# shubhamchandak94/Spring

Hardware: AMD Instinct MI355X
Metric: Mreads/s through reorder stage (higher is better)
Workload: dtype u64; 1 GPU; 100000000 x 150 bp single-end synthetic reads per GPU (uniform genome 600000000 bp, 25x coverage, 1.0% substitutions, 50% reverse-complemented), inputs resident in HBM as .dna records; reads_per_gpu=100000000, read_len=150, chains=65536, num_thr=8, parallelism=single GPU, unmatched=13958636, singletons=12720853, rounds=1984, chain_groups=2

## Files before the change

### include/spring_reorder.h

```cpp
#ifndef SPRING_REORDER_H_
#define SPRING_REORDER_H_

#include <stddef.h>
#include <stdint.h>

#ifdef __cplusplus
extern "C" {
#endif

#define SPRING_REORDER_E_ARG (-1)
#define SPRING_REORDER_E_IO (-2)
#define SPRING_REORDER_E_HIP (-3)
#define SPRING_REORDER_E_STATE (-4)

typedef struct spring_reorder_ctx spring_reorder_ctx;

typedef struct {
  int32_t device;
  uint32_t num_chains;
  int32_t num_thr;
  int32_t collect_stats;
  int32_t time_search;
  int32_t force_literal_update;
  int32_t rounds_per_sync;
// ... 10 lines not shown
  int32_t devices[8];
  int32_t mg_host_transport;
  int32_t table_mode;
  int32_t plan0[6];
  int32_t plan1[6];
  int32_t long_min;
  int32_t long_blocks;
  int32_t debug;
  int32_t long_split;
  int32_t entry_flags;
  int32_t out_writers;
  int32_t alternatives;
  int32_t phases;
  int32_t known_absent;
  int32_t sort_prefix_bits;
} spring_reorder_opts;

typedef struct {
  uint64_t n_reads, n_matched, n_single, unmatched;
  uint64_t probes, keyok, cands, hits, iterations, rounds, lost;
  uint64_t numkeys[2], dict_numreads[2];
  double ms_unpack, ms_dict, ms_chains, ms_finalize, ms_total;
  double ms_search_kernel;
  uint64_t search_launches;
  uint64_t device_bytes;
  double ms_exchange, ms_resolve_mark;
  uint64_t chains;
  uint64_t deep_pool;
  uint64_t long_searches;
  uint64_t table_minz;
  uint64_t table_marked_lines;
  uint64_t long_splits;
  uint64_t alternatives;
  uint64_t phases;
  double ms_search_busy;
  uint64_t sort_prefix_bits;
  uint64_t sort_repaired_runs;
  uint64_t sort_full_sorts;
  uint64_t sort_long_runs;
  uint64_t sort_list_overflows;
} spring_reorder_stats;

void spring_reorder_default_opts(spring_reorder_opts *o);
const char *spring_reorder_last_error(void);
void spring_reorder_trim_pool(void);

int spring_reorder_run(const char *temp_dir, uint32_t max_readlen, int32_t num_thr, int32_t paired_end,
                       uint32_t num_reads_clean_0, uint32_t num_reads_clean_1,
                       const spring_reorder_opts *opts );

int spring_reorder_create(spring_reorder_ctx **ctx, const spring_reorder_opts *opts);
void spring_reorder_destroy(spring_reorder_ctx *ctx);

int spring_reorder_load_dna(spring_reorder_ctx *ctx, const uint8_t *dna, size_t nbytes, uint32_t n,
                            uint32_t max_readlen);
// ... 82 lines not shown
```

### spring_amd/_lib.py

```python
import ctypes as C
import os

HERE = os.path.dirname(os.path.abspath(__file__))
LIB_PATH = os.environ.get("SPRING_AMD_LIB") or os.path.join(HERE, "lib", "libspring_reorder_hip.so")

EXPORTS = [
    "spring_reorder_default_opts", "spring_reorder_last_error", "spring_reorder_trim_pool", "spring_reorder_run", "spring_reorder_create",
    "spring_reorder_destroy", "spring_reorder_load_dna", "spring_reorder_load_dna_device",
    "spring_reorder_build_dict", "spring_reorder_run_chains", "spring_reorder_auto_chains", "spring_reorder_finalize",
    "spring_reorder_mg_begin", "spring_reorder_mg_search", "spring_reorder_mg_slice", "spring_reorder_mg_slices",
    "spring_reorder_mg_apply",
    "spring_reorder_mg_end", "spring_reorder_mg_exchange_virtual", "spring_reorder_debug_check_seed_state",
    "spring_mg_rccl_unique_id", "spring_mg_comm_create_rccl", "spring_mg_comm_create_host", "spring_mg_comm_destroy",
    "spring_reorder_mg_run",
    "spring_reorder_get_stats", "spring_reorder_download", "spring_reorder_tid_split", "spring_reorder_emit_dna",
    "spring_reorder_dict_lookup", "spring_reorder_download_reads", "spring_synth_dna_bytes",
    "spring_reorder_load_fastq", "spring_reorder_fastq_N",
    "spring_order_invert_se", "spring_order_invert_pe", "spring_order_correct", "spring_order_pe_encode",
    "spring_fastq_reorder",
    "spring_synth_dna_host", "spring_synth_genome_host", "spring_synth_dna_device", "spring_reorder_load_synth", "spring_reorder_download_dna",
    "spring_encoder_create", "spring_encoder_destroy", "spring_encoder_set_split_tables", "spring_encoder_encode_reorder", "spring_encoder_download",
    "spring_encoder_download_seq_packed", "spring_encoder_get_info", "spring_reorder_encode_run", "spring_encoder_encode_host", "spring_encoder_run",
]

# ... 20 lines not shown
    "spring_fastq_out_write", "spring_fastq_out_get_info",
]


class Opts(C.Structure):
    _fields_ = [("device", C.c_int32), ("num_chains", C.c_uint32), ("num_thr", C.c_int32),
                ("collect_stats", C.c_int32), ("time_search", C.c_int32), ("force_literal_update", C.c_int32),
                ("rounds_per_sync", C.c_int32), ("long_budget", C.c_int32),
                ("first_shifts", C.c_int32), ("seed_wide", C.c_int32), ("tab_scale", C.c_int32),
                ("search_wpb", C.c_int32), ("dbg_search_lds", C.c_int32), ("dbg_apply_lds", C.c_int32),
                ("fused", C.c_int32), ("deep_bins", C.c_int32),
                ("num_devices", C.c_int32), ("devices", C.c_int32 * 8), ("mg_host_transport", C.c_int32),
                ("table_mode", C.c_int32), ("plan0", C.c_int32 * 6), ("plan1", C.c_int32 * 6), ("long_min", C.c_int32),
                ("long_blocks", C.c_int32), ("debug", C.c_int32), ("long_split", C.c_int32), ("entry_flags", C.c_int32),
                ("out_writers", C.c_int32), ("alternatives", C.c_int32), ("phases", C.c_int32), ("known_absent", C.c_int32),
                ("sort_prefix_bits", C.c_int32)]


class FastqInfo(C.Structure):
    _fields_ = [("num_reads", C.c_uint32 * 2), ("num_reads_clean", C.c_uint32 * 2), ("num_reads_N", C.c_uint32 * 2),
                ("max_readlen", C.c_uint32), ("pad", C.c_uint32), ("ms_device", C.c_double)]


class EncoderInfo(C.Structure):
    _fields_ = ([(k, C.c_uint64) for k in ("n_aligned", "n_total", "seq_len", "noise_bytes", "n_noisepos",
                                           "unaligned_bytes", "len_unaligned", "num_contigs")]
                + [(k, C.c_uint32) for k in ("matched_s", "matched_N", "align_passes", "max_bin")]
                + [("ms_device", C.c_double), ("ms_phase", C.c_double * 8)])

    def asdict(self):
        d = {}
# ... 63 lines not shown
        return d


class Stats(C.Structure):
    _fields_ = ([(k, C.c_uint64) for k in ("n_reads", "n_matched", "n_single", "unmatched", "probes", "keyok",
                                          "cands", "hits", "iterations", "rounds", "lost")]
                + [("numkeys", C.c_uint64 * 2), ("dict_numreads", C.c_uint64 * 2)]
                + [(k, C.c_double) for k in ("ms_unpack", "ms_dict", "ms_chains", "ms_finalize", "ms_total",
                                             "ms_search_kernel")]
                + [("search_launches", C.c_uint64), ("device_bytes", C.c_uint64),
                   ("ms_exchange", C.c_double), ("ms_resolve_mark", C.c_double), ("chains", C.c_uint64),
                   ("deep_pool", C.c_uint64), ("long_searches", C.c_uint64),
                   ("table_minz", C.c_uint64), ("table_marked_lines", C.c_uint64), ("long_splits", C.c_uint64), ("alternatives", C.c_uint64), ("phases", C.c_uint64),
                   ("ms_search_busy", C.c_double),
                   ("sort_prefix_bits", C.c_uint64), ("sort_repaired_runs", C.c_uint64), ("sort_full_sorts", C.c_uint64),
                   ("sort_long_runs", C.c_uint64), ("sort_list_overflows", C.c_uint64)])

    def asdict(self):
        d = {}
        for k, _ in self._fields_:
            v = getattr(self, k)
            d[k] = list(v) if hasattr(v, "__len__") else v
        return d


MG_ALLGATHER_FN = C.CFUNCTYPE(C.c_int, C.c_void_p, C.c_size_t, C.c_size_t, C.c_size_t, C.c_void_p)

_lib = None


def lib():
# ... 137 lines not shown
```

### spring_amd/build.py

```python
import os
import subprocess
import sys

HERE = os.path.dirname(os.path.abspath(__file__))
ROOT = os.path.dirname(HERE)
CSRC = os.path.join(HERE, "csrc")
LIBDIR = os.path.join(HERE, "lib")
LIB = os.path.join(LIBDIR, "libspring_reorder_hip.so")
SOURCES = ["reorder_kernels.hip", "reorder_pipeline.cpp", "reorder_files.cpp", "order_ops.hip", "fastq_kernels.hip",
           "encoder.hip", "fastq_reorder.hip", "streams.hip", "decode.hip", "qualid.hip", "fastq_out.hip"]
HEADERS = ["reorder_device.h", "reorder_internal.h", "reorder_round_mc.h", "synth_common.h", "call_reorder.h",
           "encoder_internal.h", "streams_internal.h", "fastq_out_internal.h"]
PUBLIC_HEADERS = ["spring_reorder.h", "spring_encoder.h", "spring_streams.h", "spring_decode.h", "spring_qualid.h",
                  "spring_fastq_out.h"]


def _stale():
    if not os.path.exists(LIB):
        return True
    t = os.path.getmtime(LIB)
    deps = [os.path.join(CSRC, f) for f in SOURCES + HEADERS] + [os.path.join(ROOT, "include", h) for h in PUBLIC_HEADERS]
    return any(os.path.getmtime(d) > t for d in deps)


def build(force=False, verbose=False):
    if not force and not _stale():
        return LIB
# ... 28 lines not shown
```

### spring_amd/csrc/reorder_pipeline.cpp

```cpp
#include <hip/hip_runtime.h>
#include <dlfcn.h>

#include <algorithm>
#include <system_error>
#include <thread>
#include <memory>
#include <atomic>
#include <chrono>
#include <cstdarg>
#include <cstdio>
#include <cstdlib>
#include <cstring>
#include <map>
#include <mutex>
#include <new>
#include <stdexcept>
#include <string>
#include <unordered_map>
#include <vector>
#include <zlib.h>

#include "reorder_device.h"
#include "reorder_internal.h"
#include "spring_reorder.h"
#include "synth_common.h"

namespace sr {
thread_local std::string g_err;
int fail(int code, const char *fmt, ...) {
  char buf[512];
  va_list ap;
  va_start(ap, fmt);
  vsnprintf(buf, sizeof(buf), fmt, ap);
  va_end(ap);
  g_err = buf;
  return code;
}
// ... 73 lines not shown
  spring_reorder_opts o;
  int dev = 0;
  hipStream_t st = nullptr;
  int stage = ST_CREATED;
  std::vector<void *> allocs;
  uint64_t dev_bytes = 0, peak_bytes = 0;
  uint8_t *d_dna = nullptr;
  bool dna_borrowed = false;
  size_t dna_bytes = 0;
  uint64_t *d_off = nullptr;
  uint32_t n = 0;
  int L = 0, W = 0, S = 0, Lpad = 0;
  bool uniform = true;
  uint64_t *d_reads = nullptr;
  uint16_t *d_lens = nullptr;
  DictDev dict[2];
  uint4 *fpt = nullptr;
  int bshift = 63;
  int minz = 0, lshift = 31;
  uint32_t marked_lines = 0;
  bool user_plan0 = false;
  DevParams P;
  uint32_t K = 0;
  uint64_t nrec = 0, nsing = 0, cap = 0;
  bool mg = false;
  uint32_t *cnt_buf[2] = {nullptr, nullptr};
  uint64_t round_no = 0;
  hipStream_t st2 = nullptr, st3 = nullptr;
  uint64_t *taken2 = nullptr;
  uint32_t *resv2 = nullptr, *won = nullptr;
// ... 187 lines not shown
    if (p.free_blocks.empty()) continue;
    (void)hipSetDevice(d);
    for (auto &kv : p.free_blocks) { (void)hipFree(kv.second); p.sizes.erase(kv.second); }
    p.free_blocks.clear();
    p.cached = 0;
  }
}

int spring_reorder_create(spring_reorder_ctx **out, const spring_reorder_opts *opts) {
  if (!out) return fail(SPRING_REORDER_E_ARG, "ctx is NULL");
  spring_reorder_opts o;
  if (opts) o = *opts; else spring_reorder_default_opts(&o);
  if (o.num_thr <= 0) return fail(SPRING_REORDER_E_ARG, "num_thr must be >= 1");
  if (o.sort_prefix_bits < 0 || o.sort_prefix_bits > 64)
    return fail(SPRING_REORDER_E_ARG, "sort_prefix_bits: 0 (library's choice) or 1 .. 64 bits of the key hash (64 = the full sort)");
  int ndev = 0;
  HIPCHK(hipGetDeviceCount(&ndev));
  if (ndev <= 0) return fail(SPRING_REORDER_E_HIP, "no HIP device");
  int dev = o.device;
  if (dev < 0) HIPCHK(hipGetDevice(&dev));
  if (dev >= ndev) return fail(SPRING_REORDER_E_ARG, "device %d out of range (%d devices)", dev, ndev);
  HIPCHK(hipSetDevice(dev));
  spring_reorder_ctx *ctx = new spring_reorder_ctx();
  ctx->o = o;
  ctx->dev = dev;
  memset(&ctx->P, 0, sizeof(ctx->P));
  memset(&ctx->stats, 0, sizeof(ctx->stats));
  HIPCHK(hipStreamCreateWithFlags(&ctx->st, hipStreamNonBlocking));
  for (auto &e : ctx->ev) HIPCHK(hipEventCreate(&e));
  ctx->ev_ok = true;
// ... 21 lines not shown
  ctx->n = n;
  ctx->L = (int)max_readlen;
  ctx->W = (2 * ctx->L - 1) / 64 + 1;
  int S = 1;
  while (S < ctx->W) S <<= 1;
  ctx->S = S;
  ctx->Lpad = (ctx->L + 63) / 64 * 64;
  const int L = ctx->L;
  ctx->dict[0].start = L > 100 ? L / 2 - 32 : L / 2 - L * 32 / 100;
  ctx->dict[0].end = L / 2 - 1;
  ctx->dict[1].start = L / 2;
  ctx->dict[1].end = L > 100 ? L / 2 - 1 + 32 : L / 2 - 1 + L * 32 / 100;
  return 0;
}

static int unpack_on_device(spring_reorder_ctx *ctx, uint32_t *d_bad_len = nullptr) {
  if (!ctx->d_reads) DMALLOC(ctx->d_reads, (size_t)std::max<uint32_t>(ctx->n, 1) * ctx->S * sizeof(uint64_t));
  if (!ctx->d_lens) DMALLOC(ctx->d_lens, (size_t)std::max<uint32_t>(ctx->n, 1) * sizeof(uint16_t));
  HIPCHK(hipEventRecord(ctx->ev[0], ctx->st));
  const uint32_t rec = 2u + ((uint32_t)ctx->L + 3u) / 4u;
  launch_unpack(ctx->st, ctx->d_dna, ctx->d_off, ctx->n, ctx->L, ctx->W, ctx->S, rec, ctx->d_reads, ctx->d_lens, d_bad_len);
  HIPCHK(hipGetLastError());
  HIPCHK(hipEventRecord(ctx->ev[1], ctx->st));
  ctx->stage = ST_LOADED;
  return 0;
}

static int upload_chunked(spring_reorder_ctx *ctx, uint8_t *d_dst, size_t nbytes,
                          int (*fill)(void *, size_t, void *, size_t), void *self) {
  if (!nbytes) return 0;
  const size_t nchunks = (nbytes + PIN_CHUNK - 1) / PIN_CHUNK;
  const unsigned hw = std::max(1u, std::thread::hardware_concurrency());
  const int nthr = (int)std::min<size_t>(std::min<size_t>(8, hw), nchunks);
  std::atomic<size_t> next{0};
  std::atomic<int> rc{0};
  std::vector<std::string> errs((size_t)nthr);
// ... 98 lines not shown
int load_dna_source(spring_reorder_ctx *ctx, const DnaSource &src, uint32_t n, uint32_t max_readlen) {
  if (!ctx || !src.fill) return fail(SPRING_REORDER_E_ARG, "NULL argument");
  if (ctx->stage != ST_CREATED) return fail(SPRING_REORDER_E_STATE, "load_dna: context already loaded");
  HIPCHK(hipSetDevice(ctx->dev));
  int r = setup_geometry(ctx, n, max_readlen);
  if (r) return r;
  const size_t rec = 2u + (max_readlen + 3u) / 4u, nbytes = src.nbytes;
  if (n && nbytes == (size_t)n * rec) {
    ctx->uniform = true;
    ctx->dna_bytes = nbytes;
    DMALLOC(ctx->d_dna, nbytes + 16);
    if ((r = upload_chunked(ctx, ctx->d_dna, nbytes, src.fill, src.self))) return r;
    uint32_t *d_bad = nullptr, bad = 0;
    DMALLOC(d_bad, 16);
    HIPCHK(hipMemsetAsync(d_bad, 0, 4, ctx->st));
    if ((r = unpack_on_device(ctx, d_bad))) return r;
    HIPCHK(hipMemcpyAsync(&bad, d_bad, 4, hipMemcpyDeviceToHost, ctx->st));
    HIPCHK(hipStreamSynchronize(ctx->st));
    ctx->dfree(d_bad);
    if (!bad) return 0;
    ctx->stage = ST_CREATED;
    ctx->dfree(ctx->d_dna); ctx->d_dna = nullptr;
  }
  if (src.image) {
    ctx->in_source_fallback = true;
    r = spring_reorder_load_dna(ctx, src.image, nbytes, n, max_readlen);
    ctx->in_source_fallback = false;
    return r;
  }
  std::unique_ptr<uint8_t[]> img;
  try { img.reset(new uint8_t[nbytes + 1]); } catch (const std::bad_alloc &) { return fail(SPRING_REORDER_E_IO, "out of host memory for a %zu-byte record stream", nbytes); }
  {
    const size_t CH = (size_t)64 << 20, nch = (nbytes + CH - 1) / CH;
    const int nthr = (int)std::min<size_t>(std::min<size_t>(8, std::max(1u, std::thread::hardware_concurrency())), std::max<size_t>(nch, 1));
    std::atomic<size_t> next{0};
    std::atomic<int> rc{0};
// ... 56 lines not shown
    return rs;
  }
  int r = setup_geometry(ctx, n, max_readlen);
  if (r) return r;
  std::vector<uint64_t> off;
  r = scan_records(dna, nbytes, n, ctx->L, ctx->uniform, off);
  if (r) return r;
  ctx->dna_bytes = nbytes;
  DMALLOC(ctx->d_dna, nbytes + 16);
  auto mem_fill = [](void *self, size_t o, void *dst, size_t len) -> int { memcpy(dst, (const uint8_t *)self + o, len); return 0; };
  if ((r = upload_chunked(ctx, ctx->d_dna, nbytes, mem_fill, const_cast<uint8_t *>(dna)))) return r;
  if (!ctx->uniform) {
    DMALLOC(ctx->d_off, (size_t)n * sizeof(uint64_t));
    if ((r = upload_chunked(ctx, (uint8_t *)ctx->d_off, (size_t)n * sizeof(uint64_t), mem_fill, off.data()))) return r;
  }
  return unpack_on_device(ctx);
}

int spring_reorder_load_dna_device(spring_reorder_ctx *ctx, const void *d_dna, size_t nbytes, uint32_t n,
                                   uint32_t max_readlen, int32_t fixed_len) {
  if (!ctx) return fail(SPRING_REORDER_E_ARG, "ctx is NULL");
  if (ctx->stage != ST_CREATED) return fail(SPRING_REORDER_E_STATE, "load_dna_device: context already loaded");
  HIPCHK(hipSetDevice(ctx->dev));
  int r = setup_geometry(ctx, n, max_readlen);
  if (r) return r;
  if (fixed_len) {
    const size_t rec = 2u + (max_readlen + 3u) / 4u;
    if (nbytes < rec * n) return fail(SPRING_REORDER_E_ARG, "device stream too short for %u fixed records", n);
    ctx->uniform = true;
    ctx->d_dna = (uint8_t *)d_dna;
    ctx->dna_borrowed = true;
    ctx->dna_bytes = nbytes;
    return unpack_on_device(ctx);
  }
  std::vector<uint8_t> h(nbytes);
  if (nbytes) HIPCHK(hipMemcpy(h.data(), d_dna, nbytes, hipMemcpyDeviceToHost));
  return spring_reorder_load_dna(ctx, h.data(), nbytes, n, max_readlen);
}

namespace {
struct FqFile {
  uint8_t *d_txt = nullptr;
  uint64_t nbytes = 0, nlines = 0, nreads = 0;
  uint64_t *line_end = nullptr;
  uint32_t *len = nullptr, *fclean = nullptr, *szc = nullptr, *fN = nullptr, *szN = nullptr, *cidx = nullptr, *nidx = nullptr;
  uint64_t *coff = nullptr, *noff = nullptr;
  uint32_t n_clean = 0, n_N = 0, maxlen = 0, min_clean = 0xffffffffu;
  uint64_t clean_bytes = 0, N_bytes = 0;
// ... 274 lines not shown

int spring_reorder_load_synth(spring_reorder_ctx *ctx, uint32_t n, uint32_t L, uint64_t G, uint64_t seed,
                              uint32_t err_ppm) {
  if (!ctx) return fail(SPRING_REORDER_E_ARG, "ctx is NULL");
  if (ctx->stage != ST_CREATED) return fail(SPRING_REORDER_E_STATE, "load_synth: context already loaded");
  if (L == 0 || L > (uint32_t)MAX_READ_LEN || G < L) return fail(SPRING_REORDER_E_ARG, "bad synth geometry");
  if ((err_ppm & SYN_PAIRED_FLAG) && (n & 1)) return fail(SPRING_REORDER_E_ARG, "a paired pool holds an even number of reads");
  HIPCHK(hipSetDevice(ctx->dev));
  int r = setup_geometry(ctx, n, L);
  if (r) return r;
  ctx->uniform = true;
  ctx->dna_bytes = spring_synth_dna_bytes(n, L);
  DMALLOC(ctx->d_dna, ctx->dna_bytes + 16);
  launch_synth(ctx->st, ctx->d_dna, n, L, G, seed, syn_err_thr24(err_ppm));
  HIPCHK(hipGetLastError());
  return unpack_on_device(ctx);
}

int spring_reorder_download_dna(spring_reorder_ctx *ctx, uint8_t *dst, size_t cap) {
  if (!ctx || ctx->stage < ST_LOADED) return fail(SPRING_REORDER_E_STATE, "download_dna: nothing loaded");
  if (cap < ctx->dna_bytes) return fail(SPRING_REORDER_E_ARG, "buffer too small");
  HIPCHK(hipSetDevice(ctx->dev));
  HIPCHK(hipStreamSynchronize(ctx->st));
  if (ctx->dna_bytes) HIPCHK(hipMemcpy(dst, ctx->d_dna, ctx->dna_bytes, hipMemcpyDeviceToHost));
  return 0;
}

int spring_reorder_download_reads(spring_reorder_ctx *ctx, uint64_t *limbs, uint16_t *len) {
  if (!ctx || ctx->stage < ST_LOADED) return fail(SPRING_REORDER_E_STATE, "download_reads: nothing loaded");
  HIPCHK(hipSetDevice(ctx->dev));
  HIPCHK(hipStreamSynchronize(ctx->st));
// ... 30 lines not shown

int spring_reorder_build_dict(spring_reorder_ctx *ctx) {
  double t_last = now_ms();
  if (!ctx) return fail(SPRING_REORDER_E_ARG, "ctx is NULL");
  const bool dbg = ctx->o.debug != 0;
  if (ctx->stage != ST_LOADED) return fail(SPRING_REORDER_E_STATE, "build_dict: load reads first");
  HIPCHK(hipSetDevice(ctx->dev));
  hipStream_t st = ctx->st;
  const uint32_t n = ctx->n;
  HIPCHK(hipEventRecord(ctx->ev[2], st));
  uint64_t *uhash[2] = {nullptr, nullptr};
  uint32_t *ustart[2] = {nullptr, nullptr}, *ucount[2] = {nullptr, nullptr};
  const bool both_dense = n && ctx->uniform && ctx->L > ctx->dict[0].end && ctx->L > ctx->dict[1].end;
  uint64_t *keys_both[2] = {nullptr, nullptr};
  uint32_t *vals_both[2] = {nullptr, nullptr};
  ctx->stats.sort_repaired_runs = 0; ctx->stats.sort_full_sorts = 0; ctx->stats.sort_prefix_bits = 0;
  ctx->stats.sort_long_runs = 0; ctx->stats.sort_list_overflows = 0;
  for (int l = 0; l < 2; l++) {
    DictDev &d = ctx->dict[l];
    uint32_t m = 0;
    uint32_t *d_slot = nullptr, *d_flag = nullptr;
    void *d_tmp = nullptr;
    size_t tmp_bytes = 0;
    if (n) {
      if (ctx->uniform) {
        m = ctx->L > d.end ? n : 0;
      } else {
        DMALLOC(d_flag, (size_t)n * 4);
        DMALLOC(d_slot, (size_t)n * 4);
        launch_flag_in_dict(st, ctx->d_lens, n, d.end, d_flag);
// ... 17 lines not shown
      DMALLOC(d.deep, 16);
      DMALLOC(d.d_ndeep, 16);
      HIPCHK(hipMemsetAsync(d.d_ndeep, 0, 12, st));
      if (d_flag) { ctx->dfree(d_flag); ctx->dfree(d_slot); }
      continue;
    }
    uint64_t *k_in = keys_both[l], *k_out = nullptr;
    uint32_t *v_in = vals_both[l], *cnt = nullptr, *d_nruns = nullptr;
    if (!k_in) {
      DMALLOC(k_in, (size_t)m * 8);
      DMALLOC(v_in, (size_t)m * 4);
    }
    DMALLOC(k_out, (size_t)m * 8);
    DMALLOC(d.ids, (size_t)m * 4);
    DBG_T("alloc keys");
    if (l == 0 && both_dense) {
      DMALLOC(keys_both[1], (size_t)n * 8);
      DMALLOC(vals_both[1], (size_t)n * 4);
      launch_keys2(st, ctx->d_reads, n, ctx->S, d.start, d.end, ctx->dict[1].start, ctx->dict[1].end, k_in, v_in,
                   keys_both[1], vals_both[1]);
    } else if (!keys_both[l]) {
      launch_keys(st, ctx->d_reads, ctx->d_lens, ctx->uniform ? nullptr : d_slot, n, ctx->S, d.start, d.end, k_in, v_in);
    }
    HIPCHK(hipGetLastError());
    DBG_T("k_keys");
    const unsigned T = ctx->o.sort_prefix_bits > 0 ? (unsigned)ctx->o.sort_prefix_bits : sort_prefix_auto(m);
    ctx->stats.sort_prefix_bits = T;
    bool full = T >= 64;
    if (!full) {
      uint32_t *d_ctr = nullptr, *d_list = nullptr;
      uint2 *d_runs = nullptr;
// ... 59 lines not shown
    HIPCHK(hipMemsetAsync(d.d_ndeep, 0, 12, st));
    HIPCHK(hipStreamSynchronize(st));
    ctx->dfree(d_tmp);
    if (d_flag) { ctx->dfree(d_flag); ctx->dfree(d_slot); }
  }
  const uint64_t nk0 = ctx->dict[0].numkeys, nk1 = ctx->dict[1].numkeys, nm = nk0 + nk1;
  const int tab_scale = ctx->o.tab_scale > 0 ? ctx->o.tab_scale : 2;
  const uint64_t nb = std::max<uint64_t>(8, pow2ceil(std::max<uint64_t>(2, (nm * 10 + 15) / 16)) * (uint64_t)pow2ceil(tab_scale));
  ctx->bshift = 64;
  for (uint64_t v = nb; v > 1; v >>= 1) ctx->bshift--;
  ctx->minz = (ctx->dict[0].end - ctx->dict[0].start + 1 == MINZ_WL && ctx->L <= 192 && ctx->o.table_mode == 2) ? 1 : 0;
  ctx->lshift = 32 - (64 - ctx->bshift - 2);
  if (ctx->lshift < 1) return fail(SPRING_REORDER_E_ARG, "build_dict: table too large for minimizer addressing");
  ctx->stats.table_minz = ctx->minz; ctx->stats.table_marked_lines = 0;
  DMALLOC(ctx->fpt, nb * 32);
  HIPCHK(hipMemsetAsync(ctx->fpt, 0, nb * 32, st));
  uint32_t *const tab_words = reinterpret_cast<uint32_t *>(ctx->fpt);
  DBG_T("alloc+memset tab");
  if (nm) {
    uint64_t *mv0 = nullptr, *mh = nullptr, *mv = nullptr;
    void *d_tmp = nullptr;
    const uint64_t *h_in = nullptr, *v_in = nullptr;
    if (nk0 && nk1) {
      DMALLOC(mh, nm * 8);
      DMALLOC(mv, nm * 8);
      size_t tb = 0;
      HIPCHK(merge_by_hash(st, nullptr, tb, uhash[0], uhash[1], 1ull << 63, mh, mv, nk0, nk1));
      DMALLOC(d_tmp, tb);
      HIPCHK(merge_by_hash(st, d_tmp, tb, uhash[0], uhash[1], 1ull << 63, mh, mv, nk0, nk1));
      h_in = mh; v_in = mv;
    } else {
      DMALLOC(mv0, nm * 8);
      launch_iota_tag(st, mv0, nm, nk0 ? 0ull : 1ull << 63);
      h_in = nk0 ? uhash[0] : uhash[1];
// ... 1410 lines not shown
```

### spring_amd/reorder.py

```python
import ctypes as C
from dataclasses import dataclass

import numpy as np

from . import _lib


class ReorderError(RuntimeError):
    """Raised where the reference throws std::runtime_error (call_template_functions.cpp:60)."""


@dataclass
class ReorderOpts:
    device: int = -1
    num_chains: int = 0
    num_thr: int = 1
    collect_stats: bool = False
    time_search: bool = False
    force_literal_update: bool = False
    rounds_per_sync: int = 0
    first_shifts: int = 0
    seed_wide: int = 0
    tab_scale: int = 0
    search_wpb: int = 0
# ... 5 lines not shown
    devices: tuple = ()
    mg_host_transport: bool = False
    plan0: tuple = ()
    plan1: tuple = ()
    long_min: int = 0
    long_blocks: int = 0
    entry_flags: int = 0
    long_split: int = 0
    debug: bool = False
    out_writers: int = 0
    alternatives: int = 0
    table_mode: int = 0
    phases: int = 0
    known_absent: int = 0
    sort_prefix_bits: int = 0

    def to_c(self):
        o = _lib.Opts()
        _lib.lib().spring_reorder_default_opts(C.byref(o))
        o.device, o.num_chains, o.num_thr = self.device, self.num_chains, self.num_thr
        o.collect_stats, o.time_search = int(self.collect_stats), int(self.time_search)
        o.force_literal_update, o.rounds_per_sync = int(self.force_literal_update), self.rounds_per_sync
        o.first_shifts, o.seed_wide, o.tab_scale = self.first_shifts, self.seed_wide, self.tab_scale
        o.search_wpb, o.dbg_search_lds, o.dbg_apply_lds = self.search_wpb, self.dbg_search_lds, self.dbg_apply_lds
        o.fused, o.deep_bins = self.fused, self.deep_bins
        o.long_budget = self.long_budget
        if len(self.devices) > 8:
            raise ValueError("at most 8 devices")
        o.table_mode = self.table_mode
        for i, v in enumerate(tuple(self.plan0)[:6]):
            o.plan0[i] = int(v)
        for i, v in enumerate(tuple(self.plan1)[:6]):
            o.plan1[i] = int(v)
        o.long_min, o.long_blocks, o.debug = self.long_min, self.long_blocks, int(self.debug)
        o.long_split, o.entry_flags = self.long_split, self.entry_flags
        o.out_writers = self.out_writers
        o.alternatives = self.alternatives
        o.phases = self.phases
        o.known_absent = self.known_absent
        o.sort_prefix_bits = self.sort_prefix_bits
        o.num_devices = len(self.devices)
        for i, d in enumerate(self.devices):
            o.devices[i] = d
        o.mg_host_transport = int(self.mg_host_transport)
        return o


def _chk(rc):
    if rc != 0:
        raise ReorderError("%s (code %d)" % (_lib.lib().spring_reorder_last_error().decode(), rc))


class ReorderStage:

    def __init__(self, opts: ReorderOpts = None):
# ... 179 lines not shown
```

Measured before the change: 336.8 Mreads/s.

## Fuse dict key generation into unpack and build hash table in one pass

Unpacking fixed-length reads now also emits mixed dictionary keys and ids for both dictionaries in the same kernel, so the separate key-extraction pass over the unpacked reads is skipped. The fingerprint table is built by range-partitioned workgroups that assemble their bucket image in LDS and write it out whole. This replaces the memset plus merge-sort and scatter path, and buckets that run past four slots go to an overflow insert with linear probing. The cost is extra device memory held for the precomputed keys between load and build, plus a new fallback path for overflow entries.

```diff
diff --git a/include/spring_reorder.h b/include/spring_reorder.h
--- a/include/spring_reorder.h
+++ b/include/spring_reorder.h
@@ -48,6 +48,7 @@
   int32_t phases;
   int32_t known_absent;
   int32_t sort_prefix_bits;
+  int32_t dict_build_mode;
 } spring_reorder_opts;
 
 typedef struct {
@@ -73,6 +74,7 @@
   uint64_t sort_full_sorts;
   uint64_t sort_long_runs;
   uint64_t sort_list_overflows;
+  uint64_t dict_build_path;
 } spring_reorder_stats;
 
 void spring_reorder_default_opts(spring_reorder_opts *o);
diff --git a/spring_amd/_lib.py b/spring_amd/_lib.py
--- a/spring_amd/_lib.py
+++ b/spring_amd/_lib.py
@@ -58,7 +58,7 @@
                 ("table_mode", C.c_int32), ("plan0", C.c_int32 * 6), ("plan1", C.c_int32 * 6), ("long_min", C.c_int32),
                 ("long_blocks", C.c_int32), ("debug", C.c_int32), ("long_split", C.c_int32), ("entry_flags", C.c_int32),
                 ("out_writers", C.c_int32), ("alternatives", C.c_int32), ("phases", C.c_int32), ("known_absent", C.c_int32),
-                ("sort_prefix_bits", C.c_int32)]
+                ("sort_prefix_bits", C.c_int32), ("dict_build_mode", C.c_int32)]
 
 
 class FastqInfo(C.Structure):
@@ -152,7 +152,7 @@
                    ("table_minz", C.c_uint64), ("table_marked_lines", C.c_uint64), ("long_splits", C.c_uint64), ("alternatives", C.c_uint64), ("phases", C.c_uint64),
                    ("ms_search_busy", C.c_double),
                    ("sort_prefix_bits", C.c_uint64), ("sort_repaired_runs", C.c_uint64), ("sort_full_sorts", C.c_uint64),
-                   ("sort_long_runs", C.c_uint64), ("sort_list_overflows", C.c_uint64)])
+                   ("sort_long_runs", C.c_uint64), ("sort_list_overflows", C.c_uint64), ("dict_build_path", C.c_uint64)])
 
     def asdict(self):
         d = {}
diff --git a/spring_amd/build.py b/spring_amd/build.py
--- a/spring_amd/build.py
+++ b/spring_amd/build.py
@@ -8,9 +8,9 @@
 LIBDIR = os.path.join(HERE, "lib")
 LIB = os.path.join(LIBDIR, "libspring_reorder_hip.so")
 SOURCES = ["reorder_kernels.hip", "reorder_pipeline.cpp", "reorder_files.cpp", "order_ops.hip", "fastq_kernels.hip",
-           "encoder.hip", "fastq_reorder.hip", "streams.hip", "decode.hip", "qualid.hip", "fastq_out.hip"]
+           "encoder.hip", "fastq_reorder.hip", "streams.hip", "decode.hip", "qualid.hip", "fastq_out.hip", "dict_build.hip"]
 HEADERS = ["reorder_device.h", "reorder_internal.h", "reorder_round_mc.h", "synth_common.h", "call_reorder.h",
-           "encoder_internal.h", "streams_internal.h", "fastq_out_internal.h"]
+           "encoder_internal.h", "streams_internal.h", "fastq_out_internal.h", "dict_build.h"]
 PUBLIC_HEADERS = ["spring_reorder.h", "spring_encoder.h", "spring_streams.h", "spring_decode.h", "spring_qualid.h",
                   "spring_fastq_out.h"]
 
diff --git a/spring_amd/csrc/dict_build.h b/spring_amd/csrc/dict_build.h
--- /dev/null
+++ b/spring_amd/csrc/dict_build.h
@@ -0,0 +1,28 @@
+#ifndef SPRING_DICT_BUILD_H_
+#define SPRING_DICT_BUILD_H_
+
+#include "reorder_device.h"
+
+namespace sr {
+
+bool launch_unpack_keys(hipStream_t st, const uint8_t *dna, uint32_t n, int L, int W, int S, uint32_t rec_fixed,
+                        uint64_t *reads, uint16_t *lens, uint32_t *bad_len, int dstart0, int dend0, int dstart1, int dend1,
+                        uint64_t *keys0, uint32_t *vals0, uint64_t *keys1, uint32_t *vals1);
+
+constexpr int TAB_WRITE_LG = 10;
+inline int tab_write_lg(int bshift) { return 64 - bshift < TAB_WRITE_LG ? 64 - bshift : TAB_WRITE_LG; }
+inline uint32_t tab_write_blocks(int bshift) { return (uint32_t)(1ull << (64 - bshift - tab_write_lg(bshift))); }
+void launch_tab_partition(hipStream_t st, const uint64_t *h0, uint32_t nk0, const uint64_t *h1, uint32_t nk1, int bshift,
+                          uint32_t *part);
+constexpr uint32_t TAB_OVF_SLOTS = 8;
+void launch_tab_write(hipStream_t st, const uint64_t *h0, uint32_t nk0, const uint64_t *h1, uint32_t nk1,
+                      const uint32_t *part, DictBuild d0, DictBuild d1, uint4 *fpt, int bshift, uint32_t *ovf,
+                      uint32_t *ovf_blk, uint32_t *ovf_cnt);
+void launch_tab_overflow_blocks(hipStream_t st, const uint64_t *h0, uint32_t nk0, const uint64_t *h1, DictBuild d0,
+                                DictBuild d1, uint32_t *fpt, int bshift, const uint32_t *ovf_blk, const uint32_t *ovf_cnt);
+void launch_tab_overflow_pairs(hipStream_t st, const uint64_t *h0, uint32_t nk0, const uint64_t *h1, DictBuild d0,
+                               DictBuild d1, uint32_t *fpt, int bshift, const uint32_t *ovf, uint32_t novf);
+
+}
+
+#endif
diff --git a/spring_amd/csrc/dict_build.hip b/spring_amd/csrc/dict_build.hip
--- /dev/null
+++ b/spring_amd/csrc/dict_build.hip
@@ -0,0 +1,289 @@
+#include <hip/hip_runtime.h>
+
+#include "dict_build.h"
+
+namespace sr {
+
+__device__ __forceinline__ uint64_t db_mix64(uint64_t x) {
+  x ^= x >> 33; x *= 0xff51afd7ed558ccdull; x ^= x >> 33; x *= 0xc4ceb9fe1a85ec53ull; x ^= x >> 33;
+  return x;
+}
+__device__ __forceinline__ uint64_t db_unmix64(uint64_t x) {
+  x ^= x >> 33; x *= 0x9cb4b2f8129337dbull; x ^= x >> 33; x *= 0x4f74430c22a54005ull; x ^= x >> 33;
+  return x;
+}
+__device__ __forceinline__ uint32_t db_fp30_of(uint64_t h) {
+  const uint32_t f = (uint32_t)h & 0x3fffffffu;
+  return f == 0u ? 1u : f == 0x3fffffffu ? 0x3ffffffeu : f;
+}
+
+__global__ __launch_bounds__(256) void k_unpack_fixed_keys(const uint8_t *__restrict__ dna, uint32_t n, int L, int W, int lgS,
+                                                           uint32_t rec, uint64_t *__restrict__ reads,
+                                                           uint16_t *__restrict__ lens, uint32_t *__restrict__ bad_len,
+                                                           int dstart0, int klen0, int dstart1, int klen1,
+                                                           uint64_t *__restrict__ keys0, uint32_t *__restrict__ vals0,
+                                                           uint64_t *__restrict__ keys1, uint32_t *__restrict__ vals1) {
+  extern __shared__ uint4 s_unpack[];
+  const uint32_t r0 = blockIdx.x * (uint32_t)UNPACK_READS;
+  const uint32_t nr = min((uint32_t)UNPACK_READS, n - r0);
+  const uint8_t *g = dna + (uint64_t)r0 * rec;
+  const uint32_t sh = (uint32_t)((uintptr_t)g & 15u);
+  const uint4 *ga = reinterpret_cast<const uint4 *>(g - sh);
+  const uint32_t nchunk = (sh + nr * rec + 15u) >> 4;
+  for (uint32_t k = threadIdx.x; k < nchunk; k += 256) s_unpack[k] = ga[k];
+  __syncthreads();
+  const uint8_t *sb = reinterpret_cast<const uint8_t *>(s_unpack);
+  const uint32_t *sw = reinterpret_cast<const uint32_t *>(s_unpack);
+  const bool chk = bad_len != nullptr;
+  const uint32_t S = 1u << lgS;
+  auto len_of = [&](uint32_t r) -> uint32_t {
+    const uint32_t p = sh + r * rec;
+    return (uint32_t)sb[p] | ((uint32_t)sb[p + 1] << 8);
+  };
+  auto limb = [&](uint32_t m) -> uint64_t {
+    const uint32_t r = m >> lgS, j = m & (S - 1u);
+    if ((int)j >= W) return 0;
+    uint32_t len = len_of(r);
+    if (chk && len != (uint32_t)L) len = (uint32_t)L;
+    const uint32_t nb = min((len + 3u) / 4u, rec - 2u), pos = 8u * j;
+    if (pos >= nb) return 0;
+    const uint32_t p = sh + r * rec + 2u + pos, k = p >> 2, s8 = (p & 3u) * 8u;
+    uint64_t v = (uint64_t)sw[k] | ((uint64_t)sw[k + 1] << 32);
+    if (s8) v = (v >> s8) | ((uint64_t)sw[k + 2] << (64u - s8));
+    if (nb - pos < 8u) v &= (1ull << (8u * (nb - pos))) - 1ull;
+    return v;
+  };
+  for (uint32_t t = threadIdx.x; 2u * t < nr; t += 256) {
+    const uint32_t r = 2u * t;
+    uint32_t l0 = len_of(r), l1 = r + 1 < nr ? len_of(r + 1) : (uint32_t)L;
+    if (chk && (l0 != (uint32_t)L || l1 != (uint32_t)L)) {
+      *bad_len = 1u;
+      l0 = l1 = (uint32_t)L;
+    }
+    if (r + 1 < nr) *reinterpret_cast<uint32_t *>(lens + r0 + r) = l0 | (l1 << 16);
+    else lens[r0 + r] = (uint16_t)l0;
+  }
+  const uint32_t nl = nr << lgS;
+  uint64_t *out = reads + ((uint64_t)r0 << lgS);
+  for (uint32_t q = threadIdx.x; 2u * q < nl; q += 256) {
+    const uint32_t m = 2u * q;
+    const uint64_t v0 = limb(m);
+    if (m + 1 < nl) *reinterpret_cast<ulonglong2 *>(out + m) = make_ulonglong2(v0, limb(m + 1));
+    else out[m] = v0;
+  }
+  auto window = [&](uint32_t r, int dstart, int klen2) -> uint64_t {
+    const uint32_t bitpos = 2u * (uint32_t)dstart, li = bitpos >> 6, off = bitpos & 63u;
+    uint64_t v = limb((r << lgS) + li) >> off;
+    if (off && li + 1u < S) v |= limb((r << lgS) + li + 1u) << (64u - off);
+    if (klen2 < 64) v &= (1ull << klen2) - 1ull;
+    return v;
+  };
+  for (uint32_t r = threadIdx.x; r < nr; r += 256) {
+    const uint32_t i = r0 + r;
+    keys0[i] = db_mix64(window(r, dstart0, 2 * klen0));
+    vals0[i] = i;
+    keys1[i] = db_mix64(window(r, dstart1, 2 * klen1));
+    vals1[i] = i;
+  }
+}
+
+bool launch_unpack_keys(hipStream_t st, const uint8_t *dna, uint32_t n, int L, int W, int S, uint32_t rec_fixed,
+                        uint64_t *reads, uint16_t *lens, uint32_t *bad_len, int dstart0, int dend0, int dstart1, int dend1,
+                        uint64_t *keys0, uint32_t *vals0, uint64_t *keys1, uint32_t *vals1) {
+  if (!n || ((uintptr_t)reads & 15u) || ((uintptr_t)lens & 3u)) return false;
+  if (dstart0 < 0 || dstart1 < 0 || dend0 >= L || dend1 >= L || 2 * dend0 / 64 >= S || 2 * dend1 / 64 >= S) return false;
+  int lgS = 0;
+  while ((1 << lgS) < S) lgS++;
+  const size_t lds = ((size_t)UNPACK_READS * rec_fixed + 15 + 12 + 15) / 16 * 16;
+  hipLaunchKernelGGL(k_unpack_fixed_keys, dim3((n + UNPACK_READS - 1) / UNPACK_READS), dim3(256), lds, st, dna, n, L, W, lgS,
+                     rec_fixed, reads, lens, bad_len, dstart0, dend0 - dstart0 + 1, dstart1, dend1 - dstart1 + 1, keys0, vals0,
+                     keys1, vals1);
+  return true;
+}
+
+__global__ void k_tab_partition(const uint64_t *__restrict__ h0, uint32_t nk0, const uint64_t *__restrict__ h1, uint32_t nk1,
+                                int bshift, int lg, uint32_t nblk, uint32_t *__restrict__ part) {
+  const uint64_t t = (uint64_t)blockIdx.x * blockDim.x + threadIdx.x;
+  if (t >= 2ull * ((uint64_t)nblk + 1)) return;
+  const uint32_t l = t > nblk ? 1u : 0u, j = (uint32_t)(t - (l ? (uint64_t)nblk + 1 : 0));
+  const uint64_t *__restrict__ h = l ? h1 : h0;
+  const uint32_t nk = l ? nk1 : nk0;
+  uint32_t lo = 0, hi = nk;
+  if (j == nblk) {
+    lo = nk;
+  } else {
+    const uint64_t bound = ((uint64_t)j << lg) << bshift;
+    while (lo < hi) {
+      const uint32_t mid = lo + (hi - lo) / 2;
+      if (h[mid] < bound) lo = mid + 1; else hi = mid;
+    }
+  }
+  part[t] = lo;
+}
+
+constexpr uint32_t TAB_WRITE_TILE = 512, TAB_WRITE_THREADS = 512;
+__global__ __launch_bounds__(TAB_WRITE_THREADS) void k_tab_write(const uint64_t *__restrict__ h0, uint32_t nk0,
+                                                                 const uint64_t *__restrict__ h1, uint32_t nk1,
+                                                                 const uint32_t *__restrict__ part, uint32_t nblk,
+                                                                 DictBuild d0, DictBuild d1, uint4 *__restrict__ fpt,
+                                                                 int bshift, int lg, uint32_t *__restrict__ ovf,
+                                                                 uint32_t *__restrict__ ovf_blk, uint32_t *__restrict__ ovf_cnt) {
+  __shared__ uint4 img[2u << TAB_WRITE_LG];
+  __shared__ uint64_t tile[2][TAB_WRITE_TILE];
+  __shared__ uint16_t first[2][1u << TAB_WRITE_LG];
+  __shared__ uint32_t s_novf;
+  const uint32_t nbk = 1u << lg, bmask = nbk - 1u, blk = blockIdx.x;
+  for (uint32_t k = threadIdx.x; k < 2u * nbk; k += TAB_WRITE_THREADS) img[k] = make_uint4(0u, 0u, 0u, 0u);
+  for (uint32_t k = threadIdx.x; k < nbk / 2u + 1u; k += TAB_WRITE_THREADS) {
+    if (2u * k < nbk) { reinterpret_cast<uint32_t *>(first[0])[k] = 0u; reinterpret_cast<uint32_t *>(first[1])[k] = 0u; }
+  }
+  if (threadIdx.x == 0) s_novf = 0u;
+  const uint32_t a0 = part[blk], a1 = part[(uint64_t)nblk + 1 + blk];
+  const uint32_t c0 = part[blk + 1] - a0, c1 = part[(uint64_t)nblk + 2 + blk] - a1;
+  const uint32_t ntot = c0 + c1;
+  auto bin_of = [&](uint32_t t, uint32_t &st, uint32_t &cn, uint32_t &pay) {
+    const bool l = t >= c0;
+    const uint32_t i = l ? a1 + (t - c0) : a0 + t;
+    st = (l ? d1.ustart : d0.ustart)[i]; cn = (l ? d1.ucount : d0.ucount)[i];
+    pay = cn == 1u ? (l ? d1.ids : d0.ids)[st] : i;
+  };
+  uint32_t st0 = 0, cn0 = 0, pay0 = 0, st1 = 0, cn1 = 0, pay1 = 0;
+  if (threadIdx.x < ntot) bin_of(threadIdx.x, st0, cn0, pay0);
+  if (threadIdx.x + TAB_WRITE_THREADS < ntot) bin_of(threadIdx.x + TAB_WRITE_THREADS, st1, cn1, pay1);
+  __syncthreads();
+  for (uint32_t k = threadIdx.x; k < min(c0, TAB_WRITE_TILE); k += TAB_WRITE_THREADS) {
+    const uint64_t x = h0[a0 + k];
+    tile[0][k] = x;
+    if (k == 0u || (h0[a0 + k - 1u] >> bshift) != (x >> bshift)) first[0][(uint32_t)(x >> bshift) & bmask] = (uint16_t)(k + 1u);
+  }
+  for (uint32_t k = threadIdx.x; k < min(c1, TAB_WRITE_TILE); k += TAB_WRITE_THREADS) {
+    const uint64_t x = h1[a1 + k];
+    tile[1][k] = x;
+    if (k == 0u || (h1[a1 + k - 1u] >> bshift) != (x >> bshift)) first[1][(uint32_t)(x >> bshift) & bmask] = (uint16_t)(k + 1u);
+  }
+  const bool staged = c0 <= TAB_WRITE_TILE && c1 <= TAB_WRITE_TILE;
+  __syncthreads();
+  if (ntot) {
+    uint32_t *imgw = reinterpret_cast<uint32_t *>(img);
+    auto H = [&](bool l, uint32_t k) -> uint64_t {
+      if (k < TAB_WRITE_TILE) return l ? tile[1][k] : tile[0][k];
+      return l ? h1[a1 + k] : h0[a0 + k];
+    };
+    auto place = [&](uint32_t t, uint32_t st, uint32_t cn, uint32_t pay) {
+      const bool l = t >= c0;
+      const uint32_t k = l ? t - c0 : t, i = (l ? a1 : a0) + k;
+      const uint64_t hh = H(l, k), b = hh >> bshift;
+      uint32_t rank = 0;
+      while (rank < 4u && k > rank && (H(l, k - 1u - rank) >> bshift) == b) rank++;
+      if (rank < 4u && staged) {
+        const uint32_t f = l ? first[0][(uint32_t)b & bmask] : first[1][(uint32_t)b & bmask], co = l ? c0 : c1;
+        if (f) {
+          for (uint32_t o = f - 1u; rank < 4u && o < co; o++) {
+            const uint64_t x = l ? tile[0][o] : tile[1][o];
+            if ((x >> bshift) != b || (l ? x > hh : x >= hh)) break;
+            rank++;
+          }
+        }
+      } else if (rank < 4u) {
+        uint32_t lo = 0, hi = l ? c0 : c1;
+        while (lo < hi) {
+          const uint32_t mid = (lo + hi) >> 1;
+          const uint64_t x = H(!l, mid);
+          if (l ? x <= hh : x < hh) lo = mid + 1u; else hi = mid;
+        }
+        while (rank < 4u && lo > 0u && (H(!l, lo - 1u) >> bshift) == b) { rank++; lo--; }
+      }
+      uint32_t *nd = l ? d1.ndeep : d0.ndeep;
+      if (cn >= DEEP_BIN) (l ? d1.deep : d0.deep)[atomicAdd(nd, 1u)] = i;
+      if (cn >= BIG_BIN) atomicAdd(nd + 1, cn);
+      if (cn >= MID_BIN) atomicAdd(nd + 2, cn);
+      (l ? d1.urec : d0.urec)[i] = make_ulonglong2(db_unmix64(hh), (uint64_t)st | ((uint64_t)cn << 32));
+      if (rank >= 4u) {
+        const uint32_t g = l ? nk0 + i : i, slot = atomicAdd(&s_novf, 1u);
+        if (slot < TAB_OVF_SLOTS) ovf_blk[(uint64_t)blk * TAB_OVF_SLOTS + slot] = g;
+        else ovf[1u + atomicAdd(ovf, 1u)] = g;
+      } else {
+        const uint32_t bl = (uint32_t)b & bmask;
+        imgw[bl * 8u + rank] = (db_fp30_of(hh) << 2) | ((uint32_t)l << 1) | (cn == 1u ? 1u : 0u);
+        imgw[bl * 8u + 4u + rank] = pay;
+      }
+    };
+    if (threadIdx.x < ntot) place(threadIdx.x, st0, cn0, pay0);
+    if (threadIdx.x + TAB_WRITE_THREADS < ntot) place(threadIdx.x + TAB_WRITE_THREADS, st1, cn1, pay1);
+    for (uint32_t t = threadIdx.x + 2u * TAB_WRITE_THREADS; t < ntot; t += TAB_WRITE_THREADS) {
+      bin_of(t, st0, cn0, pay0);
+      place(t, st0, cn0, pay0);
+    }
+    __syncthreads();
+  }
+  if (threadIdx.x == 0) ovf_cnt[blk] = min(s_novf, TAB_OVF_SLOTS);
+  uint4 *__restrict__ out = fpt + (((uint64_t)blk << lg) << 1);
+  for (uint32_t k = threadIdx.x; k < 2u * nbk; k += TAB_WRITE_THREADS) out[k] = img[k];
+}
+
+__device__ __forceinline__ void tab_overflow_insert(uint32_t g, const uint64_t *__restrict__ h0, uint32_t nk0,
+                                                    const uint64_t *__restrict__ h1, const DictBuild &d0, const DictBuild &d1,
+                                                    uint32_t *fpt, int bshift) {
+  const uint32_t l = g >= nk0 ? 1u : 0u, u = l ? g - nk0 : g;
+  const uint64_t h = (l ? h1 : h0)[u];
+  const DictBuild &d = l ? d1 : d0;
+  const uint32_t st = d.ustart[u], cn = d.ucount[u];
+  const bool single = cn == 1u;
+  const uint32_t tag = (db_fp30_of(h) << 2) | (l << 1) | (single ? 1u : 0u);
+  const uint32_t pay = single ? d.ids[st] : u;
+  const uint64_t bmask = (1ull << (64 - bshift)) - 1;
+  uint64_t b = ((h >> bshift) + 1) & bmask;
+  for (;;) {
+    uint32_t *bk = fpt + b * 8;
+    for (int sl = 0; sl < 4; sl++) {
+      if (atomicCAS(bk + sl, 0u, tag) == 0u) {
+        bk[4 + sl] = pay;
+        return;
+      }
+    }
+    b = (b + 1) & bmask;
+  }
+}
+__global__ void k_tab_overflow_blocks(const uint64_t *__restrict__ h0, uint32_t nk0, const uint64_t *__restrict__ h1,
+                                      DictBuild d0, DictBuild d1, uint32_t *fpt, int bshift, uint32_t nblk,
+                                      const uint32_t *__restrict__ ovf_blk, const uint32_t *__restrict__ ovf_cnt) {
+  const uint64_t t = (uint64_t)blockIdx.x * blockDim.x + threadIdx.x;
+  const uint64_t blk = t / TAB_OVF_SLOTS;
+  if (blk >= nblk || (uint32_t)(t % TAB_OVF_SLOTS) >= ovf_cnt[blk]) return;
+  tab_overflow_insert(ovf_blk[t], h0, nk0, h1, d0, d1, fpt, bshift);
+}
+__global__ void k_tab_overflow_pairs(const uint64_t *__restrict__ h0, uint32_t nk0, const uint64_t *__restrict__ h1,
+                                     DictBuild d0, DictBuild d1, uint32_t *fpt, int bshift, const uint32_t *__restrict__ ovf) {
+  const uint32_t t = blockIdx.x * blockDim.x + threadIdx.x;
+  if (t >= ovf[0]) return;
+  tab_overflow_insert(ovf[1u + t], h0, nk0, h1, d0, d1, fpt, bshift);
+}
+
+void launch_tab_partition(hipStream_t st, const uint64_t *h0, uint32_t nk0, const uint64_t *h1, uint32_t nk1, int bshift,
+                          uint32_t *part) {
+  const uint32_t nblk = tab_write_blocks(bshift);
+  const uint64_t nt = 2ull * ((uint64_t)nblk + 1);
+  hipLaunchKernelGGL(k_tab_partition, dim3((unsigned)((nt + 255) / 256)), dim3(256), 0, st, h0, nk0, h1, nk1, bshift,
+                     tab_write_lg(bshift), nblk, part);
+}
+void launch_tab_write(hipStream_t st, const uint64_t *h0, uint32_t nk0, const uint64_t *h1, uint32_t nk1,
+                      const uint32_t *part, DictBuild d0, DictBuild d1, uint4 *fpt, int bshift, uint32_t *ovf,
+                      uint32_t *ovf_blk, uint32_t *ovf_cnt) {
+  const uint32_t nblk = tab_write_blocks(bshift);
+  hipLaunchKernelGGL(k_tab_write, dim3(nblk), dim3(TAB_WRITE_THREADS), 0, st, h0, nk0, h1, nk1, part, nblk, d0, d1, fpt, bshift,
+                     tab_write_lg(bshift), ovf, ovf_blk, ovf_cnt);
+}
+void launch_tab_overflow_blocks(hipStream_t st, const uint64_t *h0, uint32_t nk0, const uint64_t *h1, DictBuild d0,
+                                DictBuild d1, uint32_t *fpt, int bshift, const uint32_t *ovf_blk, const uint32_t *ovf_cnt) {
+  const uint32_t nblk = tab_write_blocks(bshift);
+  const uint64_t nt = (uint64_t)nblk * TAB_OVF_SLOTS;
+  hipLaunchKernelGGL(k_tab_overflow_blocks, dim3((unsigned)((nt + 255) / 256)), dim3(256), 0, st, h0, nk0, h1, d0, d1, fpt, bshift,
+                     nblk, ovf_blk, ovf_cnt);
+}
+void launch_tab_overflow_pairs(hipStream_t st, const uint64_t *h0, uint32_t nk0, const uint64_t *h1, DictBuild d0,
+                               DictBuild d1, uint32_t *fpt, int bshift, const uint32_t *ovf, uint32_t novf) {
+  if (!novf) return;
+  hipLaunchKernelGGL(k_tab_overflow_pairs, dim3((novf + 255) / 256), dim3(256), 0, st, h0, nk0, h1, d0, d1, fpt, bshift, ovf);
+}
+
+}
diff --git a/spring_amd/csrc/reorder_pipeline.cpp b/spring_amd/csrc/reorder_pipeline.cpp
--- a/spring_amd/csrc/reorder_pipeline.cpp
+++ b/spring_amd/csrc/reorder_pipeline.cpp
@@ -21,6 +21,7 @@
 #include <zlib.h>
 
 #include "reorder_device.h"
+#include "dict_build.h"
 #include "reorder_internal.h"
 #include "spring_reorder.h"
 #include "synth_common.h"
@@ -124,6 +125,8 @@
   bool uniform = true;
   uint64_t *d_reads = nullptr;
   uint16_t *d_lens = nullptr;
+  uint64_t *pre_keys[2] = {nullptr, nullptr};
+  uint32_t *pre_vals[2] = {nullptr, nullptr};
   DictDev dict[2];
   uint4 *fpt = nullptr;
   int bshift = 63;
@@ -341,6 +344,8 @@
   if (o.num_thr <= 0) return fail(SPRING_REORDER_E_ARG, "num_thr must be >= 1");
   if (o.sort_prefix_bits < 0 || o.sort_prefix_bits > 64)
     return fail(SPRING_REORDER_E_ARG, "sort_prefix_bits: 0 (library's choice) or 1 .. 64 bits of the key hash (64 = the full sort)");
+  if (o.dict_build_mode < 0 || o.dict_build_mode > 1)
+    return fail(SPRING_REORDER_E_ARG, "dict_build_mode: 0 (library's choice) or 1 (key pass, memset, merge and insert passes)");
   int ndev = 0;
   HIPCHK(hipGetDeviceCount(&ndev));
   if (ndev <= 0) return fail(SPRING_REORDER_E_HIP, "no HIP device");
@@ -392,12 +397,35 @@
   return 0;
 }
 
-static int unpack_on_device(spring_reorder_ctx *ctx, uint32_t *d_bad_len = nullptr) {
+static void drop_pre_keys(spring_reorder_ctx *ctx) {
+  for (int l = 0; l < 2; l++) {
+    ctx->dfree(ctx->pre_keys[l]); ctx->pre_keys[l] = nullptr;
+    ctx->dfree(ctx->pre_vals[l]); ctx->pre_vals[l] = nullptr;
+  }
+}
+
+static int unpack_on_device(spring_reorder_ctx *ctx, uint32_t *d_bad_len = nullptr, bool with_keys = false) {
   if (!ctx->d_reads) DMALLOC(ctx->d_reads, (size_t)std::max<uint32_t>(ctx->n, 1) * ctx->S * sizeof(uint64_t));
   if (!ctx->d_lens) DMALLOC(ctx->d_lens, (size_t)std::max<uint32_t>(ctx->n, 1) * sizeof(uint16_t));
+  drop_pre_keys(ctx);
+  const uint32_t rec = 2u + ((uint32_t)ctx->L + 3u) / 4u;
+  with_keys = with_keys && ctx->n && !ctx->d_off && ctx->uniform && ctx->o.dict_build_mode != 1 &&
+              ctx->L > ctx->dict[0].end && ctx->L > ctx->dict[1].end && ctx->dict[0].start >= 0;
+  if (with_keys) {
+    for (int l = 0; l < 2; l++) {
+      DMALLOC(ctx->pre_keys[l], (size_t)ctx->n * 8);
+      DMALLOC(ctx->pre_vals[l], (size_t)ctx->n * 4);
+    }
+  }
   HIPCHK(hipEventRecord(ctx->ev[0], ctx->st));
-  const uint32_t rec = 2u + ((uint32_t)ctx->L + 3u) / 4u;
-  launch_unpack(ctx->st, ctx->d_dna, ctx->d_off, ctx->n, ctx->L, ctx->W, ctx->S, rec, ctx->d_reads, ctx->d_lens, d_bad_len);
+  if (with_keys && !launch_unpack_keys(ctx->st, ctx->d_dna, ctx->n, ctx->L, ctx->W, ctx->S, rec, ctx->d_reads, ctx->d_lens, d_bad_len,
+                                       ctx->dict[0].start, ctx->dict[0].end, ctx->dict[1].start, ctx->dict[1].end,
+                                       ctx->pre_keys[0], ctx->pre_vals[0], ctx->pre_keys[1], ctx->pre_vals[1])) {
+    with_keys = false;
+    drop_pre_keys(ctx);
+  }
+  if (!with_keys)
+    launch_unpack(ctx->st, ctx->d_dna, ctx->d_off, ctx->n, ctx->L, ctx->W, ctx->S, rec, ctx->d_reads, ctx->d_lens, d_bad_len);
   HIPCHK(hipGetLastError());
   HIPCHK(hipEventRecord(ctx->ev[1], ctx->st));
   ctx->stage = ST_LOADED;
@@ -526,12 +554,13 @@
     uint32_t *d_bad = nullptr, bad = 0;
     DMALLOC(d_bad, 16);
     HIPCHK(hipMemsetAsync(d_bad, 0, 4, ctx->st));
-    if ((r = unpack_on_device(ctx, d_bad))) return r;
+    if ((r = unpack_on_device(ctx, d_bad, true))) return r;
     HIPCHK(hipMemcpyAsync(&bad, d_bad, 4, hipMemcpyDeviceToHost, ctx->st));
     HIPCHK(hipStreamSynchronize(ctx->st));
     ctx->dfree(d_bad);
     if (!bad) return 0;
     ctx->stage = ST_CREATED;
+    drop_pre_keys(ctx);
     ctx->dfree(ctx->d_dna); ctx->d_dna = nullptr;
   }
   if (src.image) {
@@ -618,7 +647,7 @@
     DMALLOC(ctx->d_off, (size_t)n * sizeof(uint64_t));
     if ((r = upload_chunked(ctx, (uint8_t *)ctx->d_off, (size_t)n * sizeof(uint64_t), mem_fill, off.data()))) return r;
   }
-  return unpack_on_device(ctx);
+  return unpack_on_device(ctx, nullptr, true);
 }
 
 int spring_reorder_load_dna_device(spring_reorder_ctx *ctx, const void *d_dna, size_t nbytes, uint32_t n,
@@ -635,7 +664,7 @@
     ctx->d_dna = (uint8_t *)d_dna;
     ctx->dna_borrowed = true;
     ctx->dna_bytes = nbytes;
-    return unpack_on_device(ctx);
+    return unpack_on_device(ctx, nullptr, true);
   }
   std::vector<uint8_t> h(nbytes);
   if (nbytes) HIPCHK(hipMemcpy(h.data(), d_dna, nbytes, hipMemcpyDeviceToHost));
@@ -940,7 +969,7 @@
   DMALLOC(ctx->d_dna, ctx->dna_bytes + 16);
   launch_synth(ctx->st, ctx->d_dna, n, L, G, seed, syn_err_thr24(err_ppm));
   HIPCHK(hipGetLastError());
-  return unpack_on_device(ctx);
+  return unpack_on_device(ctx, nullptr, true);
 }
 
 int spring_reorder_download_dna(spring_reorder_ctx *ctx, uint8_t *dst, size_t cap) {
@@ -1001,6 +1030,16 @@
   const bool both_dense = n && ctx->uniform && ctx->L > ctx->dict[0].end && ctx->L > ctx->dict[1].end;
   uint64_t *keys_both[2] = {nullptr, nullptr};
   uint32_t *vals_both[2] = {nullptr, nullptr};
+  ctx->stats.dict_build_path = 0;
+  if (both_dense && ctx->pre_keys[0] && ctx->o.dict_build_mode != 1) {
+    for (int l = 0; l < 2; l++) {
+      keys_both[l] = ctx->pre_keys[l]; vals_both[l] = ctx->pre_vals[l];
+      ctx->pre_keys[l] = nullptr; ctx->pre_vals[l] = nullptr;
+    }
+    ctx->stats.dict_build_path |= 1;
+  } else {
+    drop_pre_keys(ctx);
+  }
   ctx->stats.sort_repaired_runs = 0; ctx->stats.sort_full_sorts = 0; ctx->stats.sort_prefix_bits = 0;
   ctx->stats.sort_long_runs = 0; ctx->stats.sort_list_overflows = 0;
   for (int l = 0; l < 2; l++) {
@@ -1048,7 +1087,7 @@
     DMALLOC(k_out, (size_t)m * 8);
     DMALLOC(d.ids, (size_t)m * 4);
     DBG_T("alloc keys");
-    if (l == 0 && both_dense) {
+    if (l == 0 && both_dense && !keys_both[0]) {
       DMALLOC(keys_both[1], (size_t)n * 8);
       DMALLOC(vals_both[1], (size_t)n * 4);
       launch_keys2(st, ctx->d_reads, n, ctx->S, d.start, d.end, ctx->dict[1].start, ctx->dict[1].end, k_in, v_in,
@@ -1138,10 +1177,51 @@
   if (ctx->lshift < 1) return fail(SPRING_REORDER_E_ARG, "build_dict: table too large for minimizer addressing");
   ctx->stats.table_minz = ctx->minz; ctx->stats.table_marked_lines = 0;
   DMALLOC(ctx->fpt, nb * 32);
-  HIPCHK(hipMemsetAsync(ctx->fpt, 0, nb * 32, st));
+  const bool one_pass = nm && !ctx->minz && ctx->o.dict_build_mode != 1;
+  if (!one_pass) HIPCHK(hipMemsetAsync(ctx->fpt, 0, nb * 32, st));
   uint32_t *const tab_words = reinterpret_cast<uint32_t *>(ctx->fpt);
   DBG_T("alloc+memset tab");
-  if (nm) {
+  if (one_pass) {
+    if (nm >= 0xffffffffull) return fail(SPRING_REORDER_E_ARG, "build_dict: %llu keys exceed the 32-bit index space of the table build", (unsigned long long)nm);
+    ctx->stats.dict_build_path |= 2;
+    ctx->marked_lines = 0;
+    DictBuild db[2];
+    for (int l = 0; l < 2; l++) {
+      DictDev &d = ctx->dict[l];
+      db[l].ustart = ustart[l]; db[l].ucount = ucount[l]; db[l].ids = d.ids; db[l].urec = d.urec;
+      db[l].deep = d.deep; db[l].ndeep = d.d_ndeep;
+    }
+    uint32_t *d_part = nullptr, *d_ovf = nullptr, *d_ovf_blk = nullptr, *d_ovf_cnt = nullptr, novf = 0;
+    const size_t nblk = tab_write_blocks(ctx->bshift);
+    DMALLOC(d_part, 2 * (nblk + 1) * 4);
+    DMALLOC(d_ovf_blk, nblk * TAB_OVF_SLOTS * 4);
+    DMALLOC(d_ovf_cnt, nblk * 4);
+    DMALLOC(d_ovf, ((size_t)nm + 1) * 4);
+    HIPCHK(hipMemsetAsync(d_ovf, 0, 4, st));
+    launch_tab_partition(st, uhash[0], (uint32_t)nk0, uhash[1], (uint32_t)nk1, ctx->bshift, d_part);
+    launch_tab_write(st, uhash[0], (uint32_t)nk0, uhash[1], (uint32_t)nk1, d_part, db[0], db[1], ctx->fpt, ctx->bshift, d_ovf,
+                     d_ovf_blk, d_ovf_cnt);
+    launch_tab_overflow_blocks(st, uhash[0], (uint32_t)nk0, uhash[1], db[0], db[1], tab_words, ctx->bshift, d_ovf_blk, d_ovf_cnt);
+    HIPCHK(hipGetLastError());
+    HIPCHK(hipMemcpyAsync(&novf, d_ovf, 4, hipMemcpyDeviceToHost, st));
+    uint32_t nd[2][3] = {{0, 0, 0}, {0, 0, 0}};
+    for (int l = 0; l < 2; l++)
+      HIPCHK(hipMemcpyAsync(nd[l], ctx->dict[l].d_ndeep, 12, hipMemcpyDeviceToHost, st));
+    HIPCHK(hipStreamSynchronize(st));
+    DBG_T("table write");
+    launch_tab_overflow_pairs(st, uhash[0], (uint32_t)nk0, uhash[1], db[0], db[1], tab_words, ctx->bshift, d_ovf, novf);
+    HIPCHK(hipGetLastError());
+    for (int l = 0; l < 2; l++) { ctx->dict[l].ndeep = nd[l][0]; ctx->dict[l].big_reads = nd[l][1]; ctx->dict[l].mid_reads = nd[l][2]; }
+    if (dbg) {
+      fprintf(stderr, "[dict] %u of %llu pairs past the %u overflow slots of their workgroup\n", novf, (unsigned long long)nm, TAB_OVF_SLOTS);
+      fprintf(stderr, "[dict] reads %u + %u, keys %u + %u, bins >= %u: %u + %u, reads in bins >= %u: %u + %u, >= %u: %u + %u\n",
+              ctx->dict[0].numreads, ctx->dict[1].numreads, ctx->dict[0].numkeys, ctx->dict[1].numkeys, DEEP_BIN, nd[0][0], nd[1][0],
+              MID_BIN, nd[0][2], nd[1][2], BIG_BIN, nd[0][1], nd[1][1]);
+    }
+    ctx->stats.table_marked_lines = 0;
+    ctx->dfree(d_part); ctx->dfree(d_ovf); ctx->dfree(d_ovf_blk); ctx->dfree(d_ovf_cnt);
+    DBG_T("overflow");
+  } else if (nm) {
     uint64_t *mv0 = nullptr, *mh = nullptr, *mv = nullptr;
     void *d_tmp = nullptr;
     const uint64_t *h_in = nullptr, *v_in = nullptr;
diff --git a/spring_amd/reorder.py b/spring_amd/reorder.py
--- a/spring_amd/reorder.py
+++ b/spring_amd/reorder.py
@@ -43,6 +43,7 @@
     phases: int = 0
     known_absent: int = 0
     sort_prefix_bits: int = 0
+    dict_build_mode: int = 0
 
     def to_c(self):
         o = _lib.Opts()
@@ -68,6 +69,7 @@
         o.phases = self.phases
         o.known_absent = self.known_absent
         o.sort_prefix_bits = self.sort_prefix_bits
+        o.dict_build_mode = self.dict_build_mode
         o.num_devices = len(self.devices)
         for i, d in enumerate(self.devices):
             o.devices[i] = d
```

Result: faster. 342.0 Mreads/s, median of 6 (+1.6%).
